# YoshikiMaekawa2000/ccv_mppi_path_tracker

Hardware: AMD Instinct MI355X
Metric: trajectory rollouts/s (K×iters/s) + ms/MPPI-iteration, diff-drive T=50 (higher is better)
Workload: dtype f64; 1 GPU; C2: diff_drive K=65536 T=50 sinusoid, u_dim=2, launch parameters; samples_per_gpu=65536, horizon=50, state_store=True

## Files before the change

### ccv_mppi_path_tracker_amd/csrc/ccv_mppi_capi.hip

```cpp
#include <chrono>
#include <new>

#include "capi_internal.h"

namespace ccv {

hipError_t ensure_scratch(DeviceBuffers& d, size_t bytes) {
    if (bytes <= d.scratch_bytes) return hipSuccess;
    d.d_scratch.reset();
    d.scratch_bytes = 0;
    if (hipError_t e = d.d_scratch.alloc((bytes + sizeof(double) - 1) / sizeof(double))) return e;
    d.scratch_bytes = bytes;
    return hipSuccess;
}

void fill_params(const ccv_mppi_config& c, const bool fast_clamp_allowed, RolloutArgs& A) {
    A.sigma = c.control_noise;
    A.lambda = c.lambda;
    A.v_ref = c.v_ref;
    for (int d = 0; d < CCV_MPPI_MAX_UDIM; ++d) {
        A.umin[d] = c.u_min[d];
        A.umax[d] = c.u_max[d];
    }
    A.fast_clamp = std::isfinite(c.control_noise) ? 1 : 0;
// ... 459 lines not shown
    unpack_result(*h, h->R, h->h_pin, u_opt_out, stats);
    return CCV_MPPI_OK;
}

static int r4_prio_levels(int model) {
    auto levels = [](int noise, int dynamics, int distance, int store) { return 16 + (noise | dynamics << 2 | distance << 4 | store << 6); };
    return model == CCV_MPPI_DIFF_DRIVE ? levels(3, 2, 1, 0) : model == CCV_MPPI_STEERING_DIFF_DRIVE ? levels(2, 3, 1, 0) : levels(0, 1, 2, 3);
}

void select_kernels(KernelChoice& k, const Shape& s, const int64_t workgroups, const bool batched) {
    const int64_t cus = s.cu_count;
    const bool fb = s.cfg.model == CCV_MPPI_FULL_BODY;
    const char* kenv = getenv("CCV_MPPI_KERNEL");
    const bool coop = !(kenv && std::strcmp(kenv, "v1") == 0) && k.lds_window;
    const char* forced = batched || !coop ? nullptr : kenv;
    KernelFamily f = coop ? KernelFamily::TwoWave : KernelFamily::Plain;
    if (coop && (!fb || workgroups <= cus)) f = KernelFamily::FourWave;
    if (forced && std::strcmp(forced, "r4") == 0) f = KernelFamily::FourWave;
    if (forced && std::strcmp(forced, "r3") == 0 && !fb) f = KernelFamily::ThreeWave;
    if (forced && std::strcmp(forced, "pc") == 0) f = KernelFamily::TwoWave;
    bool solo = coop && !forced && workgroups > (fb ? (batched ? 1 : 4) : 5) * cus;
    if (forced && std::strcmp(forced, "solo") == 0) solo = true;
    k.stagewise = f;
    k.fused = solo ? KernelFamily::OneWave : f;
    k.prio_rotate = f == KernelFamily::FourWave ? r4_prio_levels(s.cfg.model) : coop ? 1 : 0;
    k.prune = (coop && s.H > 16) ? 1 : 0;
}

int check_config(const ccv_mppi_config* cfg) {
    if (cfg->abi_version != CCV_MPPI_ABI_VERSION) return CCV_MPPI_ERR_INVALID_ARG;
    if (cfg->model < CCV_MPPI_DIFF_DRIVE || cfg->model > CCV_MPPI_FULL_BODY) return CCV_MPPI_ERR_INVALID_ARG;
    if (cfg->num_samples < 1 || cfg->horizon < 3 || cfg->horizon > CCV_MPPI_MAX_HORIZON) return CCV_MPPI_ERR_INVALID_ARG;
    return CCV_MPPI_OK;
}

int check_device(const int device) {
    int ndev = 0;
    if (hipGetDeviceCount(&ndev) != hipSuccess || ndev <= 0) return CCV_MPPI_ERR_NO_DEVICE;
    if (device < 0 || device >= ndev) return CCV_MPPI_ERR_NO_DEVICE;
    return CCV_MPPI_OK;
}

void set_shape(Shape& s, const ccv_mppi_config& cfg, const int pitch, const int nblocks) {
    s.cfg = cfg;
    s.udim = udim_of(cfg.model);
    s.K = cfg.num_samples;
    s.H = cfg.horizon;
    s.R = (s.H - 1) * s.udim;
    s.pitch = pitch;
    s.nchunks = (s.K + kChunk - 1) / kChunk;
    s.nblocks = nblocks;
    hipDeviceProp_t prop;
    if (hipGetDeviceProperties(&prop, cfg.device) == hipSuccess && prop.multiProcessorCount > 0) s.cu_count = prop.multiProcessorCount;
}

int create_buffers(Core* h, const BufferCounts& n) {
    hipError_t e;
    if ((e = h->own_stream.create()) != hipSuccess) return fail(h, CCV_MPPI_ERR_HIP, "hipStreamCreate", e);
    h->stream = h->own_stream;
    const size_t P = (size_t)h->pitch;
    struct Piece { void** p; size_t bytes; } pieces[] = {
        {(void**)&h->d_z, (size_t)h->R * P * sizeof(float)},
        {(void**)&h->d_xs, (size_t)h->H * P * sizeof(double)},
        {(void**)&h->d_ys, (size_t)h->H * P * sizeof(double)},
        {(void**)&h->d_u, (size_t)h->R * P * sizeof(double)},
        {(void**)&h->d_cost, P * sizeof(double)},
        {(void**)&h->d_w, P * sizeof(double)},
        {(void**)&h->d_partial, (size_t)(h->R + 1) * n.nparts_max * sizeof(double)},
    };
    constexpr size_t kPieceAlign = (size_t)2 << 20;
    size_t arena_bytes = 0;
    for (const Piece& pc : pieces) arena_bytes += (pc.bytes + kPieceAlign - 1) / kPieceAlign * kPieceAlign;
    if ((e = h->d_arena.alloc_zeroed(arena_bytes)) != hipSuccess) return fail(h, CCV_MPPI_ERR_ALLOC, "hipMalloc", e);
    {
        size_t at = 0;
        for (const Piece& pc : pieces) {
            *pc.p = h->d_arena + at;
            at += (pc.bytes + kPieceAlign - 1) / kPieceAlign * kPieceAlign;
        }
    }
    struct { DeviceArray<double>* p; size_t n; } allocs[] = {
        {&h->d_nominal, n.nominal},
        {&h->d_nom_used, (size_t)(CCV_MPPI_MAX_HORIZON + 8) * CCV_MPPI_MAX_UDIM},
        {&h->d_statpart, n.nparts_max * 3},
        {&h->d_vec, n.vec},
        {&h->d_stats, n.stats},
        {n.extra, n.n_extra},
    };
    for (auto& a : allocs)
        if ((e = a.p->alloc_zeroed(a.n)) != hipSuccess) return fail(h, CCV_MPPI_ERR_ALLOC, "hipMalloc", e);
    if (const char* tv = std::getenv("CCV_MPPI_THROTTLE")) h->throttle = std::strcmp(tv, "0") != 0;
    for (Event& te : h->throttle_ev)
        if ((e = te.create()) != hipSuccess) return fail(h, CCV_MPPI_ERR_HIP, "creating an event", e);
    h->pin_doubles = n.pin_doubles;
    if ((e = h->h_pin.alloc(h->pin_doubles, hipHostMallocDefault)) != hipSuccess) return fail(h, CCV_MPPI_ERR_ALLOC, "hipHostMalloc", e);
    if ((e = h->h_mail.alloc(n.mail_slots * 2, hipHostMallocMapped)) != hipSuccess) return fail(h, CCV_MPPI_ERR_ALLOC, "hipHostMalloc of the mailbox", e);
    std::memset(h->h_mail, 0, n.mail_slots * 2 * sizeof(unsigned long long));
    if ((e = h->h_mail.device(&h->d_mail)) != hipSuccess) return fail(h, CCV_MPPI_ERR_HIP, "hipHostGetDevicePointer(mailbox)", e);
    if (const char* mv = std::getenv("CCV_MPPI_MAILBOX")) h->use_mail = std::strcmp(mv, "0") != 0;
    if ((e = hipDeviceSynchronize()) != hipSuccess) return fail(h, CCV_MPPI_ERR_HIP, "hipDeviceSynchronize", e);
    return CCV_MPPI_OK;
}

void wait_for_streams(Core* h) {
    if (h->stream) (void)hipStreamSynchronize(h->stream);
    if (h->own_stream && h->own_stream != h->stream) (void)hipStreamSynchronize(h->own_stream);
}

int set_stream(Core* h, void* hip_stream) {
    HIP_TRY(h, hipStreamSynchronize(h->stream));
    h->stream = hip_stream ? (hipStream_t)hip_stream : h->own_stream;
    for (bool& u : h->throttle_used) u = false;
    return CCV_MPPI_OK;
}

void track_absmax(const double* u, const size_t n, const int udim, double* absmax) {
    for (int d = 0; d < CCV_MPPI_MAX_UDIM; ++d) absmax[d] = 0.0;
    for (size_t i = 0; i < n; ++i) {
        const double a = std::fabs(u[i]), m = absmax[i % (size_t)udim];
        if (a != a || (m == m && a > m)) absmax[i % (size_t)udim] = a;
    }
}

}

extern "C" {

const char* ccv_mppi_version(void) { return "ccv_mppi_hip 0.1 (gfx950)"; }

int ccv_mppi_udim(int model) {
    if (model < CCV_MPPI_DIFF_DRIVE || model > CCV_MPPI_FULL_BODY) return CCV_MPPI_ERR_INVALID_ARG;
    return udim_of(model);
}

const char* ccv_mppi_last_error(const ccv_mppi_handle* h) { return h ? h->err.c_str() : "null handle"; }

int ccv_mppi_create(const ccv_mppi_config* cfg, ccv_mppi_handle** out) {
    if (!cfg || !out) return CCV_MPPI_ERR_INVALID_ARG;
    *out = nullptr;
    if (int rc = check_config(cfg)) return rc;
    if (cfg->sample_offset < 0 || cfg->sample_offset > INT32_MAX - cfg->num_samples) return CCV_MPPI_ERR_INVALID_ARG;
    if (int rc = check_device(cfg->device)) return rc;
    ccv_mppi_handle* h = new (std::nothrow) ccv_mppi_handle();
    if (!h) return CCV_MPPI_ERR_ALLOC;
    set_shape(*h, *cfg, round_up(cfg->num_samples, 64), (cfg->num_samples + kPcSamples - 1) / kPcSamples);
    const char* env = getenv("CCV_MPPI_WINDOW");
    h->lds_window = !(env && std::strcmp(env, "scalar") == 0);
    select_kernels(*h, *h, h->nblocks, false);
    if (const char* pv = std::getenv("CCV_MPPI_PRIO")) {
        const int v = std::atoi(pv);
        h->prio_rotate = v == 0 ? 0 : (((v >= 2 && v <= 5) || (v >= 16 && v < 16 + 256)) && h->stagewise == KernelFamily::FourWave) ? v : h->prio_rotate;
    }
    if (const char* pv = std::getenv("CCV_MPPI_PRUNE")) h->prune = std::strcmp(pv, "0") != 0;
    if (const char* pv = std::getenv("CCV_MPPI_FAST_CLAMP")) h->fast_clamp_allowed = std::strcmp(pv, "0") != 0;

    auto bail = [&](int code) {
        std::fprintf(stderr, "ccv_mppi_create: %s\n", h->err.c_str());
        ccv_mppi_destroy(h);
        return code;
    };
    const DeviceGuard guard(cfg->device);
    hipError_t e;
    if ((e = hipSetDevice(cfg->device)) != hipSuccess) return bail(fail(h, CCV_MPPI_ERR_NO_DEVICE, "hipSetDevice", e));
    const size_t nparts_max = (size_t)(h->nblocks > h->nchunks ? h->nblocks : h->nchunks);
    const size_t pad = (size_t)(CCV_MPPI_MAX_HORIZON + 8) * CCV_MPPI_MAX_UDIM;
    const size_t R = (size_t)h->R;
    if (int rc = create_buffers(h, BufferCounts{nparts_max, pad, R + 1, 4, &h->d_cmin, 1,
                                                R + 16, R + 4}))
        return bail(rc);
#if defined(CCV_DIAG)
    {
        const size_t dbg_bytes = (size_t)(kDiagHeader + kDiagSlots * kDiagBlocks) * sizeof(unsigned long long);
        if ((e = h->d_dbg.alloc_zeroed(dbg_bytes / sizeof(unsigned long long))) != hipSuccess) return bail(fail(h, CCV_MPPI_ERR_ALLOC, "hipMalloc", e));
        if ((e = hipDeviceSynchronize()) != hipSuccess) return bail(fail(h, CCV_MPPI_ERR_HIP, "hipDeviceSynchronize", e));
    }
#endif
    *out = h;
    return CCV_MPPI_OK;
}

int ccv_mppi_destroy(ccv_mppi_handle* h) {
    if (!h) return CCV_MPPI_ERR_INVALID_ARG;
    const DeviceGuard guard(h->cfg.device);
    (void)hipSetDevice(h->cfg.device);
    wait_for_streams(h);
    exchange_release(h);
    delete h;
    return CCV_MPPI_OK;
}

int ccv_mppi_set_stream(ccv_mppi_handle* h, void* hip_stream) {
    if (!h) return CCV_MPPI_ERR_INVALID_ARG;
    if (int rc = flush_pending(h)) return rc;
    return set_stream(h, hip_stream);
}

int ccv_mppi_synchronize(ccv_mppi_handle* h) {
    if (!h) return CCV_MPPI_ERR_INVALID_ARG;
    if (int rc = flush_pending(h)) return rc;
    HIP_TRY(h, hipStreamSynchronize(h->stream));
    return exchange_check(h);
}

int ccv_mppi_set_nominal(ccv_mppi_handle* h, const double* u) {
    if (!h || !u) return CCV_MPPI_ERR_INVALID_ARG;
    h->pending_vec = nullptr;
    if (int rc = flush_pending(h)) return rc;
    HIP_TRY(h, hipMemcpyAsync(h->d_nominal, u, (size_t)h->R * sizeof(double), hipMemcpyHostToDevice, h->stream));
    HIP_TRY(h, hipStreamSynchronize(h->stream));
    track_absmax(u, (size_t)h->R, h->udim, h->nom_absmax);
    return CCV_MPPI_OK;
}

int ccv_mppi_get_nominal(ccv_mppi_handle* h, double* u) {
    if (!h || !u) return CCV_MPPI_ERR_INVALID_ARG;
    if (int rc = flush_pending(h)) return rc;
    HIP_TRY(h, hipMemcpyAsync(u, h->d_nominal, (size_t)h->R * sizeof(double), hipMemcpyDeviceToHost, h->stream));
    HIP_TRY(h, hipStreamSynchronize(h->stream));
    return exchange_check(h);
}

int ccv_mppi_iterate(ccv_mppi_handle* h, const double* x0, double dt, const double* x_ref, const double* y_ref,
                     double yaw_ref0, uint64_t seed, uint64_t iter, double* u_opt_out, ccv_mppi_stats* stats) {
    int rc = check_iter_args(h, x0, dt, x_ref, y_ref);
    if (rc) return rc;
    h->want_mail = !(stats && h->timing);
    rc = enqueue_iteration(h, x0, dt, x_ref, y_ref, yaw_ref0, seed, iter, true, nullptr);
    h->want_mail = false;
    if (rc) return rc;
    return fetch_result(h, u_opt_out, stats);
}

int ccv_mppi_iterate_enqueue(ccv_mppi_handle* h, const double* x0, double dt, const double* x_ref, const double* y_ref,
                             double yaw_ref0, uint64_t seed, uint64_t iter) {
    int rc = check_iter_args(h, x0, dt, x_ref, y_ref);
    if (rc) return rc;
    return enqueue_iteration(h, x0, dt, x_ref, y_ref, yaw_ref0, seed, iter, true, nullptr);
}

int ccv_mppi_partials_size(const ccv_mppi_handle* h) { return h ? h->R + 1 : CCV_MPPI_ERR_INVALID_ARG; }

int ccv_mppi_iterate_partials_enqueue(ccv_mppi_handle* h, const double* x0, double dt, const double* x_ref,
                                      const double* y_ref, double yaw_ref0, uint64_t seed, uint64_t iter,
                                      double* dev_partials) {
    int rc = check_iter_args(h, x0, dt, x_ref, y_ref);
    if (rc) return rc;
    if (!dev_partials) return fail(h, CCV_MPPI_ERR_INVALID_ARG, "dev_partials is null");
    if (h->cfg.flags & CCV_MPPI_FLAG_MIN_SHIFT)
        return fail(h, CCV_MPPI_ERR_INVALID_ARG, "MIN_SHIFT needs a cross-device min; not supported with partials");
    return enqueue_iteration(h, x0, dt, x_ref, y_ref, yaw_ref0, seed, iter, false, dev_partials);
}

int ccv_mppi_apply_partials_enqueue(ccv_mppi_handle* h, const double* dev_partials) {
    if (!h || !dev_partials) return CCV_MPPI_ERR_INVALID_ARG;
    if (int rc = flush_pending(h)) return rc;
    h->pending_vec = dev_partials;
    return CCV_MPPI_OK;
}

}
```

### ccv_mppi_path_tracker_amd/csrc/mppi_consume.h

```cpp
#pragma once
#include "mppi_cost_terms.h"
#include "mppi_device_util.h"
#include "mppi_handoff.h"
#include "mppi_kernels.h"

namespace ccv {

constexpr int kConsumeStates = 8;

template <int NV, int NHALF, class SH>
__device__ __forceinline__ void pc_prune_window(const RolloutArgs& A, const SH& sh, const double (&px)[NV], const double (&py)[NV],
                                                const int lane, int& jb, int& je) {
    float xlo = (float)px[0], ylo = (float)py[0];
    float xhi = xlo, yhi = ylo;
#pragma unroll
    for (int i = 1; i < NV; ++i) {
        const float fx = (float)px[i], fy = (float)py[i];
        xlo = fminf(xlo, fx);
        xhi = fmaxf(xhi, fx);
        ylo = fminf(ylo, fy);
        yhi = fmaxf(yhi, fy);
    }
    wave_min_max_min_max_f32(xlo, xhi, ylo, yhi);
    const double bx0 = (double)xlo - (fabs((double)xlo) * 1.2e-7 + 1.0e-37), bx1 = (double)xhi + (fabs((double)xhi) * 1.2e-7 + 1.0e-37);
// ... 37 lines not shown
#pragma unroll
    for (int k = 0; k < 4; ++k) {
        const unsigned long long at = __ballot(mine[k] == best[k]);
        ok[k] = at != 0ull;
        const int r = ok[k] ? __builtin_ctzll(at) : 0;
        jr[k] = r + (int)((upper[k] >> r) & 1ull) * 64;
        abr[k] = sh.ab[jr[k]];
        cr[k] = sh.c[jr[k]];
    }
    unsigned long long keep[2] = {0ull, 0ull};
#pragma unroll
    for (int hh = 0; hh < NHALF; ++hh) {
        bool kp = valid[hh];
#pragma unroll
        for (int k = 0; k < 4; ++k) {
            const double da = ab[hh].x - abr[k].x, db = ab[hh].y - abr[k].y, dc = c[hh] - cr[k];
            const double L = dc + (fmin(da * bx0, da * bx1) + fmin(db * by0, db * by1));
            const double T = tj[hh] + 1.0e-9 * (fabs(cr[k]) + (fabs(abr[k].x) * X + fabs(abr[k].y) * Y));
            kp = kp && !(ok[k] && L > T);
        }
        keep[hh] = __ballot(kp);
    }
    if (keep[0] | keep[1]) {
        const int lo = keep[0] ? __builtin_ctzll(keep[0]) : 64 + __builtin_ctzll(keep[1]);
        const int hi = keep[1] ? 127 - __builtin_clzll(keep[1]) : 63 - __builtin_clzll(keep[0]);
        jb = lo & ~3;
        je = (hi | 3) + 1;
    }
}

enum ConsumeForm : unsigned { kLeanRegisters = 1u, kDiscs = 2u, kMovingDiscs = 4u };
__host__ __device__ constexpr unsigned consume_discs(const BatchForm form) {
    return form >= BatchForm::Moving ? (kDiscs | kMovingDiscs) : (form >= BatchForm::Obst ? kDiscs : 0u);
}
constexpr std::nullptr_t kNoDiscs = nullptr;
template <int NV, int MODEL, class SH, unsigned FORM = 0u>
__device__ __forceinline__ void pc_consume(const RolloutArgs& A, const SH& sh, double& cost, const int b, const int lane,
                                           int* prune_on = nullptr,
                                           const ObstLds* ob = kNoDiscs, const ObstMovLds* obm = kNoDiscs,
                                           int* taken_flag = nullptr, const int taken_value = 0) {
    constexpr bool LEAN = (FORM & kLeanRegisters) != 0, OBST = (FORM & kDiscs) != 0, MOVING = (FORM & kMovingDiscs) != 0;
    static_assert(!MOVING || OBST, "moving discs are discs");
    const int H4 = (A.H + 3) & ~3;
    double px[NV], py[NV], m[NV];
#pragma unroll
    for (int i = 0; i < NV; ++i) {
        px[i] = sh.p[b & (SH::kPBuf - 1)][i][0][lane];
        py[i] = sh.p[b & (SH::kPBuf - 1)][i][1][lane];
        if constexpr (SH::kStage) {
            px[i] -= A.x0[0];
            py[i] -= A.x0[1];
        }
        m[i] = INFINITY;
    }
    if (taken_flag) {
        asm volatile("s_waitcnt lgkmcnt(0)" ::: "memory");
        pc_publish(taken_flag, taken_value);
    }
    double2 ab0[4], ab1[4];
    double c0[4], c1[4];
    auto fetch = [&](double2(&ab)[4], double(&c)[4], const int j) {
#pragma unroll
        for (int jj = 0; jj < 4; ++jj) {
            ab[jj] = sh.ab[j + jj];
            c[jj] = sh.c[j + jj];
        }
    };
    auto points4 = [&](const double2(&ab)[4], const double(&c)[4]) {
        double f[4][NV];
#pragma unroll
        for (int jj = 0; jj < 4; ++jj)
#pragma unroll
            for (int i = 0; i < NV; ++i) f[jj][i] = fma(ab[jj].x, px[i], fma(ab[jj].y, py[i], c[jj]));
#pragma unroll
        for (int i = 0; i < NV; ++i) {
            const double t = fmin(fmin(f[0][i], f[1][i]), fmin(f[2][i], f[3][i]));
            asm("v_min_f64 %0, %1, %2" : "=v"(m[i]) : "v"(m[i]), "v"(t));
        }
    };
    int jb = 0, je = H4;
    if (A.prune && (prune_on == nullptr || *prune_on)) {
        if (H4 > 64) pc_prune_window<NV, 2>(A, sh, px, py, lane, jb, je);
        else pc_prune_window<NV, 1>(A, sh, px, py, lane, jb, je);
        if (prune_on && 4 * (je - jb) > 3 * H4) *prune_on = 0;
    }
    if constexpr (LEAN) {
        double2 qa[2], qb[2];
        double ca[2], cb[2];
        auto fetch2 = [&](double2(&ab)[2], double(&c)[2], const int j) {
            ab[0] = sh.ab[j];
            c[0] = sh.c[j];
            ab[1] = sh.ab[j + 1];
            c[1] = sh.c[j + 1];
        };
        auto points2 = [&](const double2(&ab)[2], const double(&c)[2]) {
#pragma unroll
            for (int i = 0; i < NV; ++i) {
                const double f0 = fma(ab[0].x, px[i], fma(ab[0].y, py[i], c[0]));
                const double f1 = fma(ab[1].x, px[i], fma(ab[1].y, py[i], c[1]));
                const double t = fmin(f0, f1);
                asm("v_min_f64 %0, %1, %2" : "=v"(m[i]) : "v"(m[i]), "v"(t));
            }
        };
        auto first2 = [&](const double2(&ab)[2], const double(&c)[2]) {
#pragma unroll
            for (int i = 0; i < NV; ++i) {
                const double f0 = fma(ab[0].x, px[i], fma(ab[0].y, py[i], c[0]));
                const double f1 = fma(ab[1].x, px[i], fma(ab[1].y, py[i], c[1]));
                m[i] = fmin(f0, f1);
            }
        };
        fetch2(qa, ca, jb);
        fetch2(qb, cb, jb + 2);
        __builtin_amdgcn_sched_barrier(0);
        first2(qa, ca);
        fetch2(qa, ca, jb + 4);
        __builtin_amdgcn_sched_barrier(0);
        points2(qb, cb);
        for (int j = jb + 4; j < je; j += 4) {
            fetch2(qb, cb, j + 2);
            __builtin_amdgcn_sched_barrier(0);
            points2(qa, ca);
            fetch2(qa, ca, j + 4);
            __builtin_amdgcn_sched_barrier(0);
            points2(qb, cb);
        }
    } else {
    fetch(ab0, c0, jb);
    for (int j = jb; j < je; j += 8) {
        fetch(ab1, c1, j + 4);
        __builtin_amdgcn_sched_barrier(0);
        points4(ab0, c0);
        if (j + 4 >= je) break;
        fetch(ab0, c0, j + 8);
        __builtin_amdgcn_sched_barrier(0);
        points4(ab1, c1);
    }
    }
#pragma unroll
    for (int i = 0; i < NV; ++i) {
        double d2 = m[i] + fma(px[i], px[i], py[i] * py[i]);
        if constexpr (MODEL == CCV_MPPI_FULL_BODY) {
            d2 = d2 < 1.0e4 ? fmax(d2, 0.0) : 1.0e4;
            cost += A.w_path * d2;
        } else {
            double g;
            asm("v_min_f64 %0, %1, %2" : "=v"(g) : "v"(d2), "s"(1.0e4));
            asm("v_max_f64 %0, %1, 0" : "=v"(d2) : "v"(g));
            cost = fma(A.w_path, d2, cost);
        }
    }
    if constexpr (MOVING) obst_term_moving<NV>(A, *obm, px, py, m, cost, b * kTU);
    else if constexpr (OBST) obst_term<NV>(A, *ob, px, py, m, cost);
}

template <int MODEL, class SH, unsigned FORM = 0u>
__device__ __forceinline__ void pc_consume_states(const int nv, const RolloutArgs& A, const SH& sh, double& cost, const int b, const int lane,
                                                  int* prune_on, const ObstLds* ob = kNoDiscs, const ObstMovLds* obm = kNoDiscs,
                                                  int* taken_flag = nullptr, const int taken_value = 0) {
    switch (nv) {
        case 8: pc_consume<8, MODEL, SH, FORM>(A, sh, cost, b, lane, prune_on, ob, obm, taken_flag, taken_value); break;
        case 7: pc_consume<7, MODEL, SH, FORM>(A, sh, cost, b, lane, prune_on, ob, obm, taken_flag, taken_value); break;
        case 6: pc_consume<6, MODEL, SH, FORM>(A, sh, cost, b, lane, prune_on, ob, obm, taken_flag, taken_value); break;
        case 5: pc_consume<5, MODEL, SH, FORM>(A, sh, cost, b, lane, prune_on, ob, obm, taken_flag, taken_value); break;
        case 4: pc_consume<4, MODEL, SH, FORM>(A, sh, cost, b, lane, prune_on, ob, obm, taken_flag, taken_value); break;
        case 3: pc_consume<3, MODEL, SH, FORM>(A, sh, cost, b, lane, prune_on, ob, obm, taken_flag, taken_value); break;
        case 2: pc_consume<2, MODEL, SH, FORM>(A, sh, cost, b, lane, prune_on, ob, obm, taken_flag, taken_value); break;
        case 1: pc_consume<1, MODEL, SH, FORM>(A, sh, cost, b, lane, prune_on, ob, obm, taken_flag, taken_value); break;
        default: break;
    }
}

}
```

### ccv_mppi_path_tracker_amd/csrc/mppi_kernels.h

```cpp
#pragma once
#include <hip/hip_runtime.h>
#include <math.h>
#include <stdint.h>

#include "../../include/ccv_mppi.h"

#if defined(CCV_DIAG)
#include "mppi_diag.h"
#else
#define CCV_DIAG_STAMP(A, slot) do {} while (0)
#define CCV_DIAG_STAMP_VALUE(A, slot, value) do {} while (0)
#endif

namespace ccv {

constexpr int kMaxH = CCV_MPPI_MAX_HORIZON;
constexpr int kTU = 8;
constexpr int kBlock = 256;
constexpr int kChunk = 2048;
constexpr int kPcSamples = 64;
constexpr int kPartialMin = 4;
constexpr int kMaxObst = CCV_MPPI_MAX_OBSTACLES;

enum : int { MODE_FUSED = 0, MODE_ROLLOUT = 1, MODE_COST = 2 };

enum : int { SRC_PHILOX = 0, SRC_BUFFER = 1 };

__host__ __device__ constexpr int udim_of(int model) { return model == 0 ? 2 : (model == 1 ? 3 : 5); }

struct Window {
    double a[kMaxH];
    double b[kMaxH];
    double c[kMaxH];
};

struct ResidentFrame {
    double x0[5];
    double yaw_ref0;
    int32_t index;
    int32_t steps;
    Window W;
    double x_ref[kMaxH], y_ref[kMaxH];
};

struct BatchParams;
struct BatchHead {
    double x0[5];
    double yaw_ref0;
    double dt, inv_dt;
    uint32_t seed_lo, seed_hi;
    int32_t K, k_offset;
    const double* nominal;
    const BatchParams* params;
};
struct GridRow;
struct alignas(64) BatchParams {
    double sigma, lambda, v_ref;
    double umin[5], umax[5];
    double w_path, w_v, w_zmp, w_rollv, w_back, w_yaw;
    int32_t fast_clamp, n_obst;
    const double* obst;
    double w_obs;
    const double* obst_v;
    const GridRow* grid;
};
static_assert(sizeof(BatchParams) == 192, "three 64-byte lines per instance");
struct alignas(64) GridRow {
    double origin_x, origin_y, inv, w;
    const float* cells;
    int32_t nx, ny;
    float outside;
};
static_assert(sizeof(GridRow) == 64, "one 64-byte line per instance");
enum class BatchForm : int { Single, Batch, Varied, Obst, Moving, Grid };
constexpr int kBatchHeadDoubles = 16;
__host__ __device__ constexpr int batch_record_doubles(int H) { return kBatchHeadDoubles + ((3 * H + 7) & ~7); }

struct RolloutArgs {
    double x0[5];
    double dt;
    double yaw_ref0;
    double sigma, lambda, v_ref;
    double umin[5], umax[5];
    double w_path, w_v, w_zmp, w_rollv, w_back, w_yaw;
    double fb_mass, fb_L, fb_Ixx, fb_gz;
    double inv_dt;
    uint32_t seed_lo, seed_hi, iter_lo, iter_hi;
    int32_t K, pitch, H, k_offset;
    int32_t steer_off, store_u, store_xy, do_cost;
    const double* __restrict__ nominal;
    double* u;
    float* z;
    double* nominal_used;
    double* xs;
    double* ys;
    double* cost;
    double* w;
    double* partial;
    double* statpart;
    int32_t nparts, fuse_update;
    int32_t prio_rotate, cu_count;
    int32_t prune, fast_clamp;
    const double* pending_vec;
    double* nominal_w;
    double* stats_w;
    const ResidentFrame* frame;
    unsigned long long* dbg;
};

__device__ __forceinline__ void touch_rollout_args() {
    typedef const uint32_t __attribute__((address_space(4))) * ConstArgWords;
    ConstArgWords ka = (ConstArgWords)__builtin_amdgcn_kernarg_segment_ptr();
    uint32_t t = 0;
#pragma unroll
    for (int off = 0; off < (int)sizeof(RolloutArgs); off += 64) t |= ka[off / 4];
    asm volatile("" ::"s"(t));
}

__device__ __forceinline__ RolloutArgs with_resident_pose(const RolloutArgs& Ak) {
    RolloutArgs A = Ak;
    if (Ak.frame) {
#pragma unroll
        for (int i = 0; i < 5; ++i) A.x0[i] = Ak.frame->x0[i];
        A.yaw_ref0 = Ak.frame->yaw_ref0;
    }
    return A;
}

template <bool VARIED = false>
__device__ __forceinline__ RolloutArgs batch_view(const RolloutArgs& Ak, const int inst) {
    RolloutArgs A = Ak;
    const double* rec = reinterpret_cast<const double*>(Ak.frame) + (size_t)inst * batch_record_doubles(Ak.H);
    typedef const BatchHead __attribute__((address_space(4))) * ConstHead;
    const auto& hd = *(ConstHead)(const void*)rec;
#pragma unroll
    for (int i = 0; i < 5; ++i) A.x0[i] = hd.x0[i];
    A.yaw_ref0 = hd.yaw_ref0;
    A.dt = hd.dt;
    A.inv_dt = hd.inv_dt;
    A.seed_lo = hd.seed_lo;
    A.seed_hi = hd.seed_hi;
    A.frame = reinterpret_cast<const ResidentFrame*>(rec);
    A.K = hd.K;
    A.k_offset = hd.k_offset;
    A.nominal = hd.nominal;
    if constexpr (VARIED) {
        typedef const BatchParams __attribute__((address_space(4))) * ConstParams;
        const auto& P = *(ConstParams)(const void*)hd.params;
        A.sigma = P.sigma;
        A.lambda = P.lambda;
        A.v_ref = P.v_ref;
#pragma unroll
        for (int d = 0; d < 5; ++d) {
            A.umin[d] = P.umin[d];
            A.umax[d] = P.umax[d];
        }
        A.w_path = P.w_path;
        A.w_v = P.w_v;
        A.w_zmp = P.w_zmp;
        A.w_rollv = P.w_rollv;
        A.w_back = P.w_back;
        A.w_yaw = P.w_yaw;
        A.fast_clamp = P.fast_clamp;
    }
    return A;
}
template <int MODEL, bool BATCH, bool VARIED = false>
__device__ __forceinline__ RolloutArgs rollout_view(const RolloutArgs& Ak) {
    if constexpr (BATCH) return batch_view<VARIED>(Ak, (int)blockIdx.x / ((Ak.K + 63) >> 6));
    else return with_resident_pose(Ak);
}

template <bool BATCH = false, class SH>
__device__ __forceinline__ void stage_window(const RolloutArgs& A, const Window& Wk, SH& sh, int nthreads,
                                             const int tid = threadIdx.x) {
    const int H = A.H, H4 = (H + 3) & ~3;
    if constexpr (BATCH) {
        const double* win = reinterpret_cast<const double*>(A.frame) + kBatchHeadDoubles;
        for (int j = tid; j < H4; j += nthreads) {
            sh.ab[j] = j < H ? make_double2(win[j], win[H + j]) : make_double2(0.0, 0.0);
            sh.c[j] = j < H ? win[2 * H + j] : INFINITY;
        }
    } else if (A.frame) {
        const Window& W = A.frame->W;
        for (int j = tid; j < H4; j += nthreads) {
            sh.ab[j] = j < H ? make_double2(W.a[j], W.b[j]) : make_double2(0.0, 0.0);
            sh.c[j] = j < H ? W.c[j] : INFINITY;
        }
    } else {
        for (int j = tid; j < H4; j += nthreads) {
            sh.ab[j] = j < H ? make_double2(Wk.a[j], Wk.b[j]) : make_double2(0.0, 0.0);
            sh.c[j] = j < H ? Wk.c[j] : INFINITY;
        }
    }
}

}
```

### ccv_mppi_path_tracker_amd/csrc/mppi_rollout_r4.h

```cpp
#pragma once
#include "mppi_consume.h"
#include "mppi_epilogue.h"
#include "mppi_handoff.h"
#include "mppi_produce.h"

namespace ccv {

constexpr int kR4Waves = 4;
template <int MODEL>
constexpr int kR4RB = MODEL == CCV_MPPI_FULL_BODY ? 15 : 12;

struct R4Rows {
    static constexpr int BR = 60;
    int first, n;
    __device__ __forceinline__ int count() const { return n; }
    __device__ __forceinline__ int row(const int m) const { return first + m; }
};
template <int UD>
__device__ __forceinline__ R4Rows r4_rows(const int H, const int nblocks, const int wv, int& nb_early) {
    const int R = (H - 1) * UD;
    nb_early = max(0, nblocks - 3);
    if (nb_early == 0) {
        const int per = ((R / UD + kR4Waves - 1) / kR4Waves) * UD;
        const int first = min(R, wv * per);
        return R4Rows{first, min(per, R - first)};
    }
    const int r_early = min(R, nb_early * kTU * UD);
    const int half_e = ((r_early / UD + 1) / 2) * UD, half_l = (((R - r_early) / UD + 1) / 2) * UD;
    switch (wv) {
        case 0: return R4Rows{0, half_e};
        case 1: return R4Rows{half_e, r_early - half_e};
        case 2: return R4Rows{r_early, half_l};
        default: return R4Rows{r_early + half_l, R - r_early - half_l};
    }
}
template <class T>
__device__ __forceinline__ void r4_fetch0(const RolloutArgs& A, T (&v)[kUpdCH], const R4Rows& rows, const int kk) {
    const size_t pitch = (size_t)A.pitch;
    const char* p0;
    if constexpr (std::is_same<T, float>::value) p0 = reinterpret_cast<const char*>(A.z + (size_t)rows.first * pitch);
    else p0 = reinterpret_cast<const char*>(A.u + (size_t)rows.first * pitch);
    const uint32_t koff = (uint32_t)kk * (uint32_t)sizeof(T);
#pragma unroll
    for (int i = 0; i < kUpdCH; ++i) {
        v[i] = 0;
        if (i < rows.n) v[i] = *reinterpret_cast<const T*>(p0 + (size_t)i * (pitch * sizeof(T)) + koff);
    }
}

template <int MODEL>
struct R4Shared {
    static constexpr bool kStage = true;
    static constexpr int kPBuf = 2;
    double p[2][kTU][2][kPcSamples];
    double2 ab[kMaxH + 4];
    double c[kMaxH + 4];
    float zs[2][kTU * udim_of(MODEL)][kPcSamples];
    double cost[kR4Waves][kPcSamples];
    alignas(32) double nom[(kMaxH + 8) * udim_of(MODEL)];
    int seq[8];
    int nan_seen[kR4Waves];
};

template <int MODEL, class SH>
__device__ __forceinline__ void r4_noise_block(const RolloutArgs& A, SH& sh, const int b, const int lane, const uint32_t kg) {
    pc_for_call_groups<MODEL>([&](auto C0_, auto CN_) {
        constexpr int C0 = decltype(C0_)::value, CN = decltype(CN_)::value;
        float z[4 * CN];
        pc_block_normals<MODEL, C0, CN>(A, b, kg, z);
#pragma unroll
        for (int i = 0; i < 4 * CN; ++i) sh.zs[b & 1][4 * C0 + i][lane] = z[i];
    });
}

template <int MODEL, class SH>
__device__ __forceinline__ void r4_noise_call(const RolloutArgs& A, SH& sh, const int b, const int call, const int lane, const uint32_t kg) {
    constexpr int UD = udim_of(MODEL);
    const Philox4 r = philox4x32_10(kg, (uint32_t)((b * kTU * UD) >> 2) + (uint32_t)call, A.iter_lo, A.iter_hi, A.seed_lo, A.seed_hi);
    float z[4];
    box_muller_f32(r.x, r.y, z[0], z[1]);
    box_muller_f32(r.z, r.w, z[2], z[3]);
#pragma unroll
    for (int i = 0; i < 4; ++i) sh.zs[b & 1][4 * call + i][lane] = z[i];
}

template <int MODEL, int NT>
struct R4Staged {
    static constexpr int kPerThread = ((kMaxH - 1 + kTU) * udim_of(MODEL) + NT - 1) / NT;
    double wa, wb, wc;
    double nv[kPerThread];
    double S;
};
template <int MODEL, int NT, bool BATCH = false>
__device__ __forceinline__ void r4_stage_issue(const RolloutArgs& A, const Window& Wk, const int tid, R4Staged<MODEL, NT>& L) {
    static_assert(NT >= kMaxH + 4, "one window point per thread");
    const int H = A.H, R = (H - 1) * udim_of(MODEL);
    L.wa = L.wb = 0.0;
    L.wc = INFINITY;
    if (tid < H) {
        if constexpr (BATCH) {
            const double* win = reinterpret_cast<const double*>(A.frame) + kBatchHeadDoubles;
            L.wa = win[tid];
            L.wb = win[H + tid];
            L.wc = win[2 * H + tid];
        } else if (A.frame) {
            const Window& W = A.frame->W;
            L.wa = W.a[tid];
            L.wb = W.b[tid];
            L.wc = W.c[tid];
        } else {
            L.wa = Wk.a[tid];
            L.wb = Wk.b[tid];
            L.wc = Wk.c[tid];
        }
    }
    const double* src = A.pending_vec ? A.pending_vec + 1 : A.nominal;
    L.S = A.pending_vec ? A.pending_vec[0] : 1.0;
#pragma unroll
    for (int i = 0; i < R4Staged<MODEL, NT>::kPerThread; ++i) {
        const int j = tid + i * NT;
        L.nv[i] = j < R ? src[j] : 0.0;
    }
}
template <int MODEL, int NT, class SH>
__device__ __forceinline__ bool r4_stage_commit(const RolloutArgs& A, SH& sh, const int tid, const R4Staged<MODEL, NT>& L) {
    const int H = A.H, H4 = (H + 3) & ~3, R = (H - 1) * udim_of(MODEL);
    if (tid < H4) {
        sh.ab[tid] = make_double2(L.wa, L.wb);
        sh.c[tid] = L.wc;
    }
    bool bad = false;
#pragma unroll
    for (int i = 0; i < R4Staged<MODEL, NT>::kPerThread; ++i) {
        const int j = tid + i * NT;
        if (j < R + kTU * udim_of(MODEL)) {
            const double v = (A.pending_vec && j < R) ? L.nv[i] / L.S : L.nv[i];
            sh.nom[j] = v;
            bad |= v != v;
            if (blockIdx.x == 0 && j < R) {
                if (A.pending_vec) A.nominal_w[j] = v;
                A.nominal_used[j] = v;
            }
        }
    }
    if (A.pending_vec && blockIdx.x == 0 && tid == 0) A.stats_w[0] = L.S;
    return bad;
}

struct R4Lane {
    int lane, k, kk;
    bool live;
    uint32_t kg;
};
template <bool FRESH>
__device__ __forceinline__ R4Lane r4_lane(const RolloutArgs& A) {
    R4Lane L;
    if constexpr (FRESH) {
        uint32_t none = 0u;
        asm volatile("" : "+v"(none));
        L.lane = (int)__builtin_amdgcn_mbcnt_hi(~0u, __builtin_amdgcn_mbcnt_lo(~0u, none));
    } else {
        L.lane = (int)__builtin_amdgcn_mbcnt_hi(~0u, __builtin_amdgcn_mbcnt_lo(~0u, 0u));
        asm volatile("" : "+v"(L.lane));
    }
    L.k = (int)blockIdx.x * kPcSamples + L.lane;
    L.live = L.k < A.K;
    L.kk = L.live ? L.k : A.K - 1;
    L.kg = (uint32_t)(A.k_offset + L.kk);
    return L;
}

struct R4ClampInLoop {
    bool fast;
};
template <class C, class F>
__device__ __forceinline__ void r4_with_clamp(const C c, F&& f) {
    if constexpr (std::is_same<C, R4ClampInLoop>::value) {
        if (c.fast) f(std::true_type{});
        else f(std::false_type{});
    } else {
        f(c);
    }
}
template <class B>
constexpr unsigned r4_clamp_flag(B) {
    return B::value ? kFastClamp : 0u;
}

template <int MODEL, int MODE, bool WIDE = false, bool TAIL = false, BatchForm FORM = BatchForm::Single, bool SHIFT = false>
__global__ __launch_bounds__(kR4Waves * 64, MODEL == CCV_MPPI_FULL_BODY ? 1 : 4) void k_rollout_r4(const RolloutArgs Ak, const Window Wk) {
    constexpr bool BATCH = FORM >= BatchForm::Batch, VARIED = FORM >= BatchForm::Varied, OBST = FORM >= BatchForm::Obst,
                   MOVING = FORM >= BatchForm::Moving, GRID = FORM >= BatchForm::Grid;
    constexpr bool FB = MODEL == CCV_MPPI_FULL_BODY;
    constexpr bool COST = MODE != MODE_ROLLOUT;
    constexpr int UD = udim_of(MODEL);
    constexpr bool kFreshLane = MODE == MODE_FUSED;
    static_assert(!WIDE || (MODEL == CCV_MPPI_DIFF_DRIVE && MODE == MODE_FUSED), "the wide-turn form exists for the fused diff-drive iteration");
    static_assert(!TAIL || MODE == MODE_FUSED, "the stage-wise modes carry the masked producer anyway");
    static_assert(!BATCH || MODE == MODE_FUSED, "batch handles run the fused iteration only");
    static_assert(!SHIFT || VARIED, "the shifted weights are built on the per-instance-parameter kernels");
    static_assert(!OBST || MODE == MODE_FUSED, "the obstacle term is the fused iteration's");
    __shared__ R4Shared<MODEL> sh;
    ObstLds* obst_lds = nullptr;
    ObstMovLds* obst_mov = nullptr;
    if constexpr (MOVING) {
        __shared__ ObstMovLds s_obst_mov;
        obst_mov = &s_obst_mov;
    } else if constexpr (OBST) {
        __shared__ ObstLds s_obst;
        obst_lds = &s_obst;
    }
    static_assert(offsetof(R4Shared<MODEL>, zs) + sizeof(sh.zs) >= kR4Waves * kR4RB<MODEL> * (kPcSamples + 2) * sizeof(double), "epilogue buffers");
    touch_rollout_args();
    const RolloutArgs A = rollout_view<MODEL, BATCH, VARIED>(Ak);
    if (A.prio_rotate) pc_set_priority((int)blockIdx.x / A.cu_count);
    const int H = A.H;
    const int wv = __builtin_amdgcn_readfirstlane(threadIdx.x >> 6);
    if (wv == 0) CCV_DIAG_STAMP(A, 0);
    const int nblocks = (H + kTU - 1) / kTU;
    const int nstates = FB ? H - 2 : H;
    const int nfull = MODE == MODE_FUSED ? (TAIL ? (H - 1 + kTU - kPartialMin) / kTU : (H - 1) / kTU) : 0;
    int* const seq_noise = &sh.seq[0];
    if (threadIdx.x < 8) sh.seq[threadIdx.x] = (threadIdx.x == 0 && nfull > 0) ? 1 : 0;
    PcState<MODEL> S;
    bool bad_nominal = false;
    if constexpr (MODE == MODE_FUSED) {
        R4Staged<MODEL, kR4Waves * 64> staged;
        r4_stage_issue<MODEL, kR4Waves * 64, BATCH>(A, Wk, (int)threadIdx.x, staged);
        if (nfull > 0) {
            constexpr int NCALL = kTU * UD / 4;
            const R4Lane L = r4_lane<kFreshLane>(A);
            for (int c = wv; c < NCALL; c += kR4Waves) r4_noise_call<MODEL>(A, sh, 0, c, L.lane, L.kg);
        }
        if (wv == 0) CCV_DIAG_STAMP(A, 3);
        if (wv == 1) {
            pc_initial_state<MODEL>(A, S);
            CCV_DIAG_STAMP(A, 1);
        }
        bad_nominal = r4_stage_commit<MODEL>(A, sh, (int)threadIdx.x, staged);
        if constexpr (OBST) {
            const int j = (int)threadIdx.x - 2 * 64;
            if (j >= 0 && j < kMaxObst) obst_stage_form<FORM>(A, obst_lds, obst_mov, j);
        }
        const bool wave_bad = __builtin_amdgcn_ballot_w64(bad_nominal) != 0ull;
        if (r4_lane<kFreshLane>(A).lane == 0) sh.nan_seen[wv] = wave_bad ? 1 : 0;
    } else {
        if constexpr (COST) stage_window(A, Wk, sh, kR4Waves * 64);
        if (wv == 1) pc_initial_state<MODEL>(A, S);
    }
    __syncthreads();
    if (wv == 1) CCV_DIAG_STAMP(A, 2);
    const bool fast_clamp = MODE == MODE_FUSED && A.fast_clamp &&
                            __builtin_amdgcn_readfirstlane(sh.nan_seen[0] | sh.nan_seen[1] | sh.nan_seen[2] | sh.nan_seen[3]) == 0;
    int* const seq_ready = &sh.seq[1];
    int* const seq_dist = &sh.seq[2];
    int* const seq_store = &sh.seq[3];
    int* const seq_stored = &sh.seq[4];
    int nb_early;
    R4Rows rows = r4_rows<UD>(H, nblocks, wv, nb_early);
    if (!(COST && A.fuse_update)) rows.n = 0;
    UpdT<MODE> upd[kUpdCH];
    auto early_fetch = [&]() {
        if constexpr (MODE == MODE_FUSED) {
            if (rows.n > 0 && nb_early > 0) {
                pc_wait_for(seq_stored, nb_early);
                r4_fetch0(A, upd, rows, r4_lane<kFreshLane>(A).kk);
            }
        }
    };
    if (wv == 0) {
        if constexpr (MODE == MODE_FUSED) {
            const R4Lane L = r4_lane<kFreshLane>(A);
            const int lane = L.lane;
            const uint32_t kg = L.kg;
            for (int b = 1; b < nfull; ++b) {
                r4_rotate_priority(A, b, 0);
                if (b >= 2) {
                    pc_wait_for(seq_ready, b - 1);
                    pc_wait_for(seq_store, b - 1);
                }
                r4_noise_block<MODEL>(A, sh, b, lane, kg);
                pc_publish(seq_noise, b + 1);
            }
            CCV_DIAG_STAMP(A, 15);
        }
        if constexpr (COST) sh.cost[0][r4_lane<kFreshLane>(A).lane] = 0.0;
        if (A.prio_rotate) __builtin_amdgcn_s_setprio(0);
        early_fetch();
    } else if (wv == 1) {
        R4Lane L;
        if constexpr (MODE != MODE_FUSED) L = r4_lane<kFreshLane>(A);
        double cost = 0.0;
        cost += pc_initial_cost<MODEL, MODE>(A);
        auto blocks = [&](auto CLAMP_) {
            constexpr unsigned LDSZ = kNormalsInLds | (WIDE ? kWideTurn : 0u);
            auto opened = [&](const int b) {
                r4_rotate_priority(A, b, 1);
                if (b >= 2) {
                    pc_wait_for(seq_dist, b - 1);
                    pc_wait_for(seq_store, b - 1);
                }
                return min(kTU, H - 1 - b * kTU);
            };
            auto closed = [&](const int b) {
                pc_publish(seq_ready, b + 1);
                if (b == 0) CCV_DIAG_STAMP(A, 5);
            };
            if constexpr (MODE == MODE_FUSED) {
                const int lane = r4_lane<kFreshLane>(A).lane;
                auto noise_fed = [&](const int b) {
                    const int nctl = opened(b);
                    pc_wait_for(seq_noise, b + 1);
                    if (b == 0) CCV_DIAG_STAMP(A, 4);
                    return nctl;
                };
                const int nwhole = (TAIL && nfull > 0 && H - 1 - (nfull - 1) * kTU < kTU) ? nfull - 1 : nfull;
                for (int b = 0; b < nwhole; ++b) {
                    noise_fed(b);
                    r4_with_clamp(CLAMP_, [&](auto FAST_) {
                        pc_produce_batched<MODEL, MODE, R4Shared<MODEL>, LDSZ | r4_clamp_flag(FAST_)>(A, sh, S, cost, b, lane, 0, 0, false, 0u);
                    });
                    closed(b);
                }
                if constexpr (TAIL) {
                    if (nwhole < nfull) {
                        const int b = nwhole, nctl = noise_fed(b);
                        r4_with_clamp(CLAMP_, [&](auto FAST_) {
                            constexpr unsigned LP = LDSZ | kPartialBlock | r4_clamp_flag(FAST_);
                            if (decltype(FAST_)::value && nctl == 6)
                                pc_produce_batched<MODEL, MODE, R4Shared<MODEL>, LP, 6>(A, sh, S, cost, b, lane, 0, 0, false, 0u, kNoNormalsAhead, nctl);
                            else
                                pc_produce_batched<MODEL, MODE, R4Shared<MODEL>, LP>(A, sh, S, cost, b, lane, 0, 0, false, 0u, kNoNormalsAhead, nctl);
                        });
                        closed(b);
                    }
                }
            }
            if constexpr (MODE == MODE_FUSED) L = r4_lane<kFreshLane>(A);
            const int lane = L.lane, k = L.k, kk = L.kk;
            const bool live = L.live;
            const uint32_t kg = L.kg;
            for (int b = nfull; b < nblocks; ++b) {
                const int nctl = opened(b);
                if (MODE != MODE_FUSED && nctl == kTU) {
                    pc_produce_batched<MODEL, MODE>(A, sh, S, cost, b, lane, k, kk, live, kg);
                } else if (MODE != MODE_FUSED && nctl >= kPartialMin) {
                    pc_produce_batched<MODEL, MODE, R4Shared<MODEL>, kPartialBlock>(A, sh, S, cost, b, lane, k, kk, live, kg, kNoNormalsAhead, nctl);
                } else {
                    pc_produce<MODEL, MODE, false>(A, sh, S, cost, b, lane, k, kk, live, kg);
                }
                closed(b);
            }
        };
        if constexpr (MODE == MODE_FUSED && !FB) {
            if (fast_clamp) blocks(std::true_type{});
            else blocks(std::false_type{});
        } else {
            blocks(R4ClampInLoop{fast_clamp});
        }
        CCV_DIAG_STAMP(A, 6);
        if constexpr (COST) sh.cost[1][L.lane] = cost;
        if (A.prio_rotate) __builtin_amdgcn_s_setprio(0);
        early_fetch();
    } else if (wv == 2) {
        int prune_on = 1;
        const int lane = r4_lane<kFreshLane>(A).lane;
        double cost = 0.0;
        for (int b = 0; b < nblocks; ++b) {
            r4_rotate_priority(A, b, 2);
            pc_wait_for(seq_ready, b + 1);
            bool taken = false;
            if constexpr (COST) {
                const int nv = min(kConsumeStates, nstates - b * kTU);
                taken = nv > 0;
                pc_consume_states<MODEL, R4Shared<MODEL>, kLeanRegisters | consume_discs(FORM)>(nv, A, sh, cost, b, lane, &prune_on, obst_lds, obst_mov, seq_dist, b + 1);
            }
            if (!taken) pc_publish(seq_dist, b + 1);
            if (b == 0) CCV_DIAG_STAMP(A, 14);
        }
        CCV_DIAG_STAMP(A, 7);
        if constexpr (COST) sh.cost[2][lane] = cost;
    } else {
        const size_t pitch = (size_t)A.pitch;
        const R4Lane L = r4_lane<kFreshLane>(A);
        const int lane = L.lane;
        const uint32_t koff4 = (uint32_t)L.k * 4u, koff8 = (uint32_t)L.k * 8u;
        GridAcc grid_acc{};
        if constexpr (GRID) grid_acc = GridAcc{grid_row(A), 0.0, nstates, nullptr};
        for (int b = 0; b < nblocks; ++b) {
            r4_rotate_priority(A, b, 3);
            pc_wait_for(seq_ready, b + 1);
            const int t0 = b * kTU;
            float zv[kTU * UD];
            double xv[kTU], yv[kTU];
            if constexpr (MODE == MODE_FUSED) {
#pragma unroll
                for (int r = 0; r < kTU * UD; ++r) zv[r] = sh.zs[b & 1][r][lane];
            }
            if constexpr (MODE != MODE_COST) {
#pragma unroll
                for (int tt = 0; tt < kTU; ++tt) {
                    xv[tt] = sh.p[b & 1][tt][0][lane];
                    yv[tt] = sh.p[b & 1][tt][1][lane];
                }
            }
            asm volatile("s_waitcnt lgkmcnt(0)" ::: "memory");
            pc_publish(seq_store, b + 1);
            GridTap tap[kTU];
            if constexpr (GRID) {
                grid_issue(grid_acc, xv, yv, tap);
            }
            if constexpr (MODE == MODE_FUSED) {
                const int nrows = min(kTU, H - 1 - t0) * UD;
                char* const zrow = reinterpret_cast<char*>(A.z + (size_t)(t0 * UD) * pitch);
                static_for<kTU * UD>([&](auto RR) {
                    constexpr int r = decltype(RR)::value;
                    if (r < nrows) pc_store_f32(zrow + (size_t)r * (pitch * 4), koff4, zv[r]);
                });
            }
            if constexpr (MODE != MODE_COST) {
                if (A.store_xy) {
                    const int nst = min(kTU, H - t0);
                    char* const xrow = reinterpret_cast<char*>(A.xs + (size_t)t0 * pitch);
                    char* const yrow = reinterpret_cast<char*>(A.ys + (size_t)t0 * pitch);
#pragma unroll
                    for (int tt = 0; tt < kTU; ++tt) {
                        if (tt < nst) {
                            pc_store_f64_stream(xrow + (size_t)tt * (pitch * 8), koff8, xv[tt]);
                            pc_store_f64_stream(yrow + (size_t)tt * (pitch * 8), koff8, yv[tt]);
                        }
                    }
                }
            }
            if constexpr (GRID) {
                grid_sum(grid_acc, tap, t0);
            }
            if constexpr (MODE == MODE_FUSED) {
                constexpr int kRowsZ = kTU * UD, kRowsAll = kTU * UD + 2 * kTU;
                static_assert(kRowsAll <= 63, "vmcnt is a 6-bit counter");
                if (t0 + kTU <= H - 1 && A.store_xy) asm volatile("s_waitcnt vmcnt(%0)" ::"n"(kRowsAll) : "memory");
                else if (t0 + kTU <= H - 1) asm volatile("s_waitcnt vmcnt(%0)" ::"n"(kRowsZ) : "memory");
                else asm volatile("s_waitcnt vmcnt(0)" ::: "memory");
                pc_publish(seq_stored, b);
            }
        }
        asm volatile("s_waitcnt vmcnt(0)" ::: "memory");
        if constexpr (GRID) sh.cost[3][lane] = grid_acc.G;
        else if constexpr (COST) sh.cost[3][lane] = 0.0;
    }
    if (A.prio_rotate) __builtin_amdgcn_s_setprio(0);
    if constexpr (COST) {
        const int R = (H - 1) * UD;
        const int mcount = rows.n;
        const R4Lane L = r4_lane<kFreshLane>(A);
        const int lane = L.lane, k = L.k, kk = L.kk;
        const bool live = L.live;
        pc_barrier_lds();
        if (wv == 0) CCV_DIAG_STAMP(A, 8);
        bool from_lds = false;
        if constexpr (MODE == MODE_FUSED) {
            from_lds = nblocks <= 2;
            if (from_lds) {
                constexpr int kMaxLdsRows = 4 * UD;
                static_assert(kMaxLdsRows <= kUpdCH, "first chunk");
#pragma unroll
                for (int i = 0; i < kMaxLdsRows; ++i) {
                    const int row = rows.first + min(i, max(mcount - 1, 0));
                    upd[i] = sh.zs[(row / (kTU * UD)) & 1][row % (kTU * UD)][lane];
                }
                pc_barrier_lds();
            }
        }
        if (!from_lds && (MODE != MODE_FUSED || wv >= 2 || nb_early == 0) && mcount > 0) r4_fetch0(A, upd, rows, kk);
        double total_;
        if constexpr (GRID) {
            total_ = ((sh.cost[0][lane] + sh.cost[1][lane]) + sh.cost[2][lane]) + 0.0;
            const ConstGridRow g = grid_row(A);
            if (g) total_ = fma(g->w, sh.cost[3][lane], total_);
        } else {
            total_ = ((sh.cost[0][lane] + sh.cost[1][lane]) + sh.cost[2][lane]) + sh.cost[3][lane];
        }
        const double total = total_;
        double wgt_;
        if constexpr (SHIFT) wgt_ = pc_shifted_weight(A, total, live);
        else wgt_ = live ? exp(-total / A.lambda) : 0.0;
        const double wgt = wgt_;
        if (wv == 0 && live) {
            A.cost[k] = total;
            A.w[k] = wgt;
        }
        if (wv == 0) CCV_DIAG_STAMP_VALUE(A, 9, wgt);
        if (wv == 2) CCV_DIAG_STAMP_VALUE(A, 11, wgt);
        if (A.fuse_update) {
            double* buf = &sh.p[0][0][0][0] + wv * (kR4RB<MODEL> * (kPcSamples + 2));
            pc_reduce_rows<kR4RB<MODEL>, MODEL, true>(A, sh, buf, upd, rows, mcount, wgt, lane, kk, fast_clamp);
            if (wv == kR4Waves - 1) pc_block_stats(A, R, wgt, total, live, lane);
        }
        if (wv == 0) CCV_DIAG_STAMP(A, 10);
        if (wv == 2) CCV_DIAG_STAMP(A, 12);
        if (wv == 3) CCV_DIAG_STAMP(A, 13);
    }
}

}
```

Measured before the change: 1.888 billion rollouts/s.

## Share tail path-cost consumption across idle noise and dynamics waves

Once production finishes, the noise and dynamics waves (0 and 1) sit idle while the distance wave works through the last blocks' path-distance terms. This change hands part of the last one or two blocks' states to waves 0 and 1. They compute the clamped squared distances into reused LDS noise slots and signal through new sequence flags, and wave 2 folds those values into its cost. Early fetch of the update is deferred until after the shared work. This adds extra synchronisation and an LDS aliasing risk. It is enabled by default whenever pruning is on.

```diff
diff --git a/ccv_mppi_path_tracker_amd/csrc/ccv_mppi_capi.hip b/ccv_mppi_path_tracker_amd/csrc/ccv_mppi_capi.hip
--- a/ccv_mppi_path_tracker_amd/csrc/ccv_mppi_capi.hip
+++ b/ccv_mppi_path_tracker_amd/csrc/ccv_mppi_capi.hip
@@ -635,6 +635,8 @@
         h->prio_rotate = v == 0 ? 0 : (((v >= 2 && v <= 5) || (v >= 16 && v < 16 + 256)) && h->stagewise == KernelFamily::FourWave) ? v : h->prio_rotate;
     }
     if (const char* pv = std::getenv("CCV_MPPI_PRUNE")) h->prune = std::strcmp(pv, "0") != 0;
+    const char* share = std::getenv("CCV_MPPI_DRAIN_SHARE");
+    if (h->prune && !(share && std::strcmp(share, "0") == 0)) h->prune |= kPruneDrainShare;
     if (const char* pv = std::getenv("CCV_MPPI_FAST_CLAMP")) h->fast_clamp_allowed = std::strcmp(pv, "0") != 0;
 
     auto bail = [&](int code) {
diff --git a/ccv_mppi_path_tracker_amd/csrc/mppi_consume.h b/ccv_mppi_path_tracker_amd/csrc/mppi_consume.h
--- a/ccv_mppi_path_tracker_amd/csrc/mppi_consume.h
+++ b/ccv_mppi_path_tracker_amd/csrc/mppi_consume.h
@@ -213,6 +213,66 @@
     }
     if constexpr (MOVING) obst_term_moving<NV>(A, *obm, px, py, m, cost, b * kTU);
     else if constexpr (OBST) obst_term<NV>(A, *ob, px, py, m, cost);
+}
+
+template <int NV, int MODEL, class SH>
+__device__ __forceinline__ void pc_consume_d2(const RolloutArgs& A, const SH& sh, const int b, const int i0, const int lane, double (&d2)[NV]) {
+    static_assert(MODEL != CCV_MPPI_FULL_BODY && SH::kStage, "the path term of diff drive and steering, staged absolute positions");
+    const int H4 = (A.H + 3) & ~3;
+    double px[NV], py[NV], m[NV];
+#pragma unroll
+    for (int i = 0; i < NV; ++i) {
+        px[i] = sh.p[b & (SH::kPBuf - 1)][i0 + i][0][lane] - A.x0[0];
+        py[i] = sh.p[b & (SH::kPBuf - 1)][i0 + i][1][lane] - A.x0[1];
+    }
+    int jb = 0, je = H4;
+    if (A.prune) {
+        if (H4 > 64) pc_prune_window<NV, 2>(A, sh, px, py, lane, jb, je);
+        else pc_prune_window<NV, 1>(A, sh, px, py, lane, jb, je);
+    }
+    double2 qa[2], qb[2];
+    double ca[2], cb[2];
+    auto fetch2 = [&](double2(&ab)[2], double(&c)[2], const int j) {
+        ab[0] = sh.ab[j];
+        c[0] = sh.c[j];
+        ab[1] = sh.ab[j + 1];
+        c[1] = sh.c[j + 1];
+    };
+    auto pair_min = [&](const double2(&ab)[2], const double(&c)[2], const int i) {
+        const double f0 = fma(ab[0].x, px[i], fma(ab[0].y, py[i], c[0]));
+        const double f1 = fma(ab[1].x, px[i], fma(ab[1].y, py[i], c[1]));
+        return fmin(f0, f1);
+    };
+    auto points2 = [&](const double2(&ab)[2], const double(&c)[2]) {
+#pragma unroll
+        for (int i = 0; i < NV; ++i) {
+            const double t = pair_min(ab, c, i);
+            asm("v_min_f64 %0, %1, %2" : "=v"(m[i]) : "v"(m[i]), "v"(t));
+        }
+    };
+    fetch2(qa, ca, jb);
+    fetch2(qb, cb, jb + 2);
+    __builtin_amdgcn_sched_barrier(0);
+#pragma unroll
+    for (int i = 0; i < NV; ++i) m[i] = pair_min(qa, ca, i);
+    fetch2(qa, ca, jb + 4);
+    __builtin_amdgcn_sched_barrier(0);
+    points2(qb, cb);
+    for (int j = jb + 4; j < je; j += 4) {
+        fetch2(qb, cb, j + 2);
+        __builtin_amdgcn_sched_barrier(0);
+        points2(qa, ca);
+        fetch2(qa, ca, j + 4);
+        __builtin_amdgcn_sched_barrier(0);
+        points2(qb, cb);
+    }
+#pragma unroll
+    for (int i = 0; i < NV; ++i) {
+        const double s = m[i] + fma(px[i], px[i], py[i] * py[i]);
+        double g;
+        asm("v_min_f64 %0, %1, %2" : "=v"(g) : "v"(s), "s"(1.0e4));
+        asm("v_max_f64 %0, %1, 0" : "=v"(d2[i]) : "v"(g));
+    }
 }
 
 template <int MODEL, class SH, unsigned FORM = 0u>
diff --git a/ccv_mppi_path_tracker_amd/csrc/mppi_kernels.h b/ccv_mppi_path_tracker_amd/csrc/mppi_kernels.h
--- a/ccv_mppi_path_tracker_amd/csrc/mppi_kernels.h
+++ b/ccv_mppi_path_tracker_amd/csrc/mppi_kernels.h
@@ -75,6 +75,8 @@
 enum class BatchForm : int { Single, Batch, Varied, Obst, Moving, Grid };
 constexpr int kBatchHeadDoubles = 16;
 __host__ __device__ constexpr int batch_record_doubles(int H) { return kBatchHeadDoubles + ((3 * H + 7) & ~7); }
+
+constexpr int32_t kPruneOn = 1, kPruneDrainShare = 2;
 
 struct RolloutArgs {
     double x0[5];
diff --git a/ccv_mppi_path_tracker_amd/csrc/mppi_rollout_r4.h b/ccv_mppi_path_tracker_amd/csrc/mppi_rollout_r4.h
--- a/ccv_mppi_path_tracker_amd/csrc/mppi_rollout_r4.h
+++ b/ccv_mppi_path_tracker_amd/csrc/mppi_rollout_r4.h
@@ -61,6 +61,60 @@
     int seq[8];
     int nan_seen[kR4Waves];
 };
+
+struct R4Deal {
+    int b, i0, n;
+};
+struct R4Drain {
+    bool on;
+    int dist_n0, dist_n1;
+    R4Deal noise;
+    R4Deal dyn0, dyn1;
+};
+constexpr int kDrainMaxShare = 3;
+__device__ __forceinline__ R4Drain r4_drain(const int nblocks, const int nstates, const bool enabled) {
+    R4Drain d{};
+    d.on = enabled && nblocks >= 3;
+    if (!d.on) return d;
+    const int last = nblocks - 1, nv_last = nstates - last * kTU;
+    if (nv_last <= 3) {
+        d.dist_n0 = 3;
+        d.dist_n1 = 0;
+        d.noise = R4Deal{last - 1, 3, 3};
+        d.dyn0 = R4Deal{last - 1, 6, 2};
+        d.dyn1 = R4Deal{last, 0, nv_last};
+    } else {
+        const int n0 = (nv_last + 2) / 3, n1 = (nv_last - n0 + 1) / 2;
+        d.dist_n0 = kTU;
+        d.dist_n1 = n0;
+        d.noise = R4Deal{last, n0, n1};
+        d.dyn0 = R4Deal{last, n0 + n1, nv_last - n0 - n1};
+        d.dyn1 = R4Deal{last, 0, 0};
+    }
+    return d;
+}
+template <class SH>
+__device__ __forceinline__ double* r4_drain_slots(SH& sh, const int nblocks) {
+    static_assert(sizeof(sh.zs[0]) >= kTU * kPcSamples * sizeof(double) && offsetof(SH, zs) % 8 == 0 && sizeof(sh.zs[0]) % 8 == 0, "8 slots of 64 doubles");
+    return reinterpret_cast<double*>(&sh.zs[(nblocks - 2) & 1][0][0]);
+}
+template <int MODEL, class SH>
+__device__ __forceinline__ void r4_drain_task(const RolloutArgs& A, SH& sh, double* const slots, const R4Deal t, const int lane) {
+    auto states = [&](auto NV_) {
+        constexpr int NV = decltype(NV_)::value;
+        double d2[NV];
+        pc_consume_d2<NV, MODEL, SH>(A, sh, t.b, t.i0, lane, d2);
+#pragma unroll
+        for (int i = 0; i < NV; ++i) slots[(t.i0 + i) * kPcSamples + lane] = d2[i];
+    };
+    static_assert(kDrainMaxShare == 3, "one case per share");
+    switch (t.n) {
+        case 3: states(std::integral_constant<int, 3>{}); break;
+        case 2: states(std::integral_constant<int, 2>{}); break;
+        case 1: states(std::integral_constant<int, 1>{}); break;
+        default: break;
+    }
+}
 
 template <int MODEL, class SH>
 __device__ __forceinline__ void r4_noise_block(const RolloutArgs& A, SH& sh, const int b, const int lane, const uint32_t kg) {
@@ -256,6 +310,8 @@
     int* const seq_dist = &sh.seq[2];
     int* const seq_store = &sh.seq[3];
     int* const seq_stored = &sh.seq[4];
+    constexpr bool DRAIN = MODE == MODE_FUSED && !FB && FORM == BatchForm::Single;
+    auto drain_of_launch = [&]() { return r4_drain(nblocks, nstates, (A.prune & (kPruneOn | kPruneDrainShare)) == (kPruneOn | kPruneDrainShare)); };
     int nb_early;
     R4Rows rows = r4_rows<UD>(H, nblocks, wv, nb_early);
     if (!(COST && A.fuse_update)) rows.n = 0;
@@ -286,7 +342,7 @@
         }
         if constexpr (COST) sh.cost[0][r4_lane<kFreshLane>(A).lane] = 0.0;
         if (A.prio_rotate) __builtin_amdgcn_s_setprio(0);
-        early_fetch();
+        if constexpr (!DRAIN) early_fetch();
     } else if (wv == 1) {
         R4Lane L;
         if constexpr (MODE != MODE_FUSED) L = r4_lane<kFreshLane>(A);
@@ -361,7 +417,7 @@
         CCV_DIAG_STAMP(A, 6);
         if constexpr (COST) sh.cost[1][L.lane] = cost;
         if (A.prio_rotate) __builtin_amdgcn_s_setprio(0);
-        early_fetch();
+        if constexpr (!DRAIN) early_fetch();
     } else if (wv == 2) {
         int prune_on = 1;
         const int lane = r4_lane<kFreshLane>(A).lane;
@@ -371,12 +427,32 @@
             pc_wait_for(seq_ready, b + 1);
             bool taken = false;
             if constexpr (COST) {
-                const int nv = min(kConsumeStates, nstates - b * kTU);
+                int nv = min(kConsumeStates, nstates - b * kTU);
+                if constexpr (DRAIN) {
+                    if (b >= nblocks - 2) {
+                        const R4Drain d = drain_of_launch();
+                        if (d.on) nv = b == nblocks - 2 ? d.dist_n0 : d.dist_n1;
+                    }
+                }
                 taken = nv > 0;
                 pc_consume_states<MODEL, R4Shared<MODEL>, kLeanRegisters | consume_discs(FORM)>(nv, A, sh, cost, b, lane, &prune_on, obst_lds, obst_mov, seq_dist, b + 1);
             }
             if (!taken) pc_publish(seq_dist, b + 1);
             if (b == 0) CCV_DIAG_STAMP(A, 14);
+        }
+        if constexpr (DRAIN && COST) {
+            const R4Drain d = drain_of_launch();
+            if (d.on) {
+                const double* const slots = r4_drain_slots(sh, nblocks);
+                auto add = [&](int* const flag, const int value, const R4Deal t) {
+                    if (t.n == 0) return;
+                    pc_wait_for(flag, value);
+                    for (int i = t.i0; i < t.i0 + t.n; ++i) cost = fma(A.w_path, slots[i * kPcSamples + lane], cost);
+                };
+                add(&sh.seq[5], 1, d.noise);
+                add(&sh.seq[6], 1, d.dyn0);
+                add(&sh.seq[6], 2, d.dyn1);
+            }
         }
         CCV_DIAG_STAMP(A, 7);
         if constexpr (COST) sh.cost[2][lane] = cost;
@@ -448,6 +524,24 @@
         if constexpr (GRID) sh.cost[3][lane] = grid_acc.G;
         else if constexpr (COST) sh.cost[3][lane] = 0.0;
     }
+    if constexpr (DRAIN && COST) {
+        if (wv < 2) {
+            const R4Drain d = drain_of_launch();
+            if (d.on) {
+                double* const slots = r4_drain_slots(sh, nblocks);
+                const int lane = r4_lane<kFreshLane>(A).lane;
+                pc_wait_for(seq_store, nblocks - 1);
+                for (int i = 0; i < 2; ++i) {
+                    const R4Deal t = wv == 0 ? (i == 0 ? d.noise : R4Deal{0, 0, 0}) : (i == 0 ? d.dyn0 : d.dyn1);
+                    if (t.n == 0) break;
+                    pc_wait_for(seq_ready, t.b + 1);
+                    r4_drain_task<MODEL>(A, sh, slots, t, lane);
+                    pc_publish(&sh.seq[5 + wv], i + 1);
+                }
+            }
+            early_fetch();
+        }
+    }
     if (A.prio_rotate) __builtin_amdgcn_s_setprio(0);
     if constexpr (COST) {
         const int R = (H - 1) * UD;
```

New measurement: 1.824 billion rollouts/s. 0.966x the previous value.
